# brunohs1993/Nanokappa

Measured on AMD Instinct MI355X. Metric: phonon-steps/sec (whole node), higher is better.
Workload: dtype f64

## Files before the change

nanokappa_amd/csrc/nk_engine.hip:

```cpp
#include <hip/hip_runtime.h>
#include <dlfcn.h>
#include <math.h>
#include <stdio.h>
#include <stdlib.h>
#include <string.h>
#include <algorithm>
#include <functional>
#include <queue>
#include <string>
#include <type_traits>
#include <chrono>
#include <time.h>
#include <vector>

#include <rccl/rccl.h>

#include "../../include/nanokappa_hip.h"
#include "nk_kernels.h"
#include "nk_field.h"
#include "nk_modes.h"
#include "nk_group.h"
#include "nk_freepath.h"
#include "nk_freecols.h"
#ifndef NK_PLAIN_IN_ENGINE
// ... 1957 lines not shown
}

static size_t nk_events_lds(nk_ctx *ctx, size_t lds_g) {
    NkDev &d = ctx->d;
    size_t lds_ev = lds_g;
    if (!(d.qx && nk_geom_mode(ctx) == 2 && d.NG > 0 && d.tree_nfam > 0)) return lds_ev;
    const size_t off = (lds_g + 15) & ~(size_t)15, fixed = off + (size_t)NK_EVENTS_PEND * NK_EV_WG * 4 + 1024;
    size_t budget = (size_t)160 * 1024 / NK_EV_PER_CU > fixed ? (size_t)160 * 1024 / NK_EV_PER_CU - fixed : 0;
    if (const char *e = getenv("NK_EVENTS_TREE_LDS")) { const size_t v = (size_t)atol(e); if (v < budget) budget = v; }
    for (int l = 0; l <= d.tree_top; ++l) {
        const int fam0 = d.tree_base[l] >> 2;
        const size_t bytes = (size_t)(d.tree_nfam - fam0) * NK_TREE_FAMILY_FLOATS * 4;
        if (bytes <= budget) { d.tree_lds_fam0 = fam0; d.tree_lds_off = (int32_t)off; lds_ev = off + bytes; break; }
    }
    if (getenv("NK_VERBOSE") && ctx->timing.batches <= 1)
        fprintf(stderr, "[nanokappa_hip] k_events: families %d .. %d of the face tree in LDS (%zu B of %zu B per workgroup)\n", d.tree_lds_fam0, d.tree_nfam, lds_ev - off, lds_ev);
    return lds_ev;
}
static int nk_side_tallies(nk_ctx *ctx, int s, std::vector<int> &band_s) {
    const int64_t stepno = ctx->step + s;
    if (!nk_flux_step(ctx, stepno)) return NK_OK;
    const int nranks = ctx->comm ? ctx->comm_nranks : 1;
    if (ctx->band_B > 0) {
        NK_TRY(nk_band_pass(ctx, false, ctx->band_rows_d + band_s.size() * 4 * (size_t)ctx->d.S * ctx->band_B));
        band_s.push_back(s);
    }
    if (ctx->field.on && nk_nth_step(ctx->field.cfg.every, stepno)) {
        NK_TRY(nk_field_sample(ctx, false, false));
        NK_HIP(nk_field_accumulate(ctx->field.g, ctx->field, nranks, ctx->stream));
        if (ctx->fgroups.on) {
            NK_TRY(nk_field_sample(ctx, true, false));
            NK_HIP(nk_field_accumulate(ctx->fgroups.g, ctx->field, nranks, ctx->stream));
        }
    }
    if (ctx->modes.on && nk_nth_step(ctx->modes.cfg.every, stepno)) {
        NK_TRY(nk_modes_sample(ctx, false));
        NK_HIP(nk_modes_accumulate(ctx->modes, nranks, ctx->num_cu, ctx->stream));
    }
    return NK_OK;
}
static int nk_band_collect(nk_ctx *ctx, const std::vector<int> &band_s, int32_t nd) {
    if (band_s.empty()) return NK_OK;
    const size_t rl = 4 * (size_t)ctx->d.S * ctx->band_B;
    std::vector<double> br(band_s.size() * rl);
    NK_HIP(hipMemcpyAsync(br.data(), ctx->band_rows_d, br.size() * sizeof(double), hipMemcpyDeviceToHost, ctx->stream));
    NK_HIP(hipStreamSynchronize(ctx->stream));
    const int unseen = ctx->halt_words[2] ? nd - 1 : -1;
    for (size_t r = 0; r < band_s.size(); ++r) {
        if (band_s[r] >= nd || band_s[r] == unseen) continue;
        ctx->band_rows.insert(ctx->band_rows.end(), br.begin() + r * rl, br.begin() + (r + 1) * rl);
        ctx->band_steps.push_back(ctx->step + band_s[r]);
    }
    return NK_OK;
}
static int nk_batch_timing(nk_ctx *ctx, int nev, int32_t nsteps, int32_t nd) {
    const hipEvent_t *ev = ctx->evpool.data();
    float ms = 0.f;
    double sk = 0.0, ek = 0.0, vk = 0.0;
    const int nt = nd < nev ? nd : nev;
    for (int s = 0; s < nt; ++s) {
        NK_HIP(hipEventElapsedTime(&ms, ev[4 * s], ev[4 * s + 1])); ek += ms;
        NK_HIP(hipEventElapsedTime(&ms, ev[4 * s + 1], ev[4 * s + 2])); sk += ms;
        NK_HIP(hipEventElapsedTime(&ms, ev[4 * s + 2], ev[4 * s + 3])); vk += ms;
    }
    NK_HIP(hipEventElapsedTime(&ms, ev[64], ev[65]));
    if (nt > 0 && nd == nsteps) {
        ctx->timing.step_kernel_ms = sk / nt;
        ctx->timing.emit_kernel_ms = ek / nt;
        ctx->timing.events_kernel_ms = vk / nt;
        ctx->timing.total_ms = ms;
    }
    return NK_OK;
}
#ifdef NK_STAMPS
#include "nk_stamps.h"
#endif

static int nk_step_batch(nk_ctx *ctx, int32_t nsteps, std::vector<double> &h, int32_t *done) {
    NkDev &d = ctx->d;
    const int R = d.R, NB = d.NB;
    NkBatch b;
    NK_TRY(nk_batch_enter(ctx, nsteps, b));
    const size_t lds_g = nk_lds(ctx, true), lds_w = nk_lds(ctx, true, d.pid ? 3 : 2), lds_e = nk_lds(ctx, true, 1);
    const size_t lds_t = lds_e > (size_t)(NK_WG * 8 + 16) ? lds_e : (size_t)(NK_WG * 8 + 16);
    const size_t lds_ev = nk_events_lds(ctx, lds_g);
    const int gm_ = nk_geom_mode(ctx);
    const bool rough_ = d.Fr > 0, rbf_ = d.sv_interp == 3, pid_ = (bool)d.pid, split_ = d.qx != nullptr;
    const bool lrec_ = nk_want_lrec(ctx);
    const int g_sweep = b.g_sweep, g_emit = b.g_emit;
    const int g_ev = split_ ? ctx->num_cu * NK_EV_PER_CU : 0;
    const int rows = g_sweep + g_ev;
    const int nev = nsteps < 4 ? 0 : 4;
    NK_TRY(nk_batch_events(ctx));
    hipEvent_t *ev = ctx->evpool.data();
    NK_HIP(hipEventRecord(ev[64], ctx->stream));
    std::vector<int> band_s;
    if (ctx->band_B > 0) {
        int nflux = 0;
        for (int s = 0; s < nsteps; ++s) nflux += nk_flux_step(ctx, ctx->step + s) ? 1 : 0;
        if (nflux > 0) NK_TRY(nk_band_ensure(ctx, nflux));
    }
    for (int s = 0; s < nsteps; ++s) {
        NK_TRY(nk_batch_prelude(ctx, b, s));
        const NkGroupRec rec = nk_batch_rec(ctx, b, s);
        const uint32_t step = rec.step;
        const int do_flux = rec.do_flux;
        if (s < nev) NK_HIP(hipEventRecord(ev[4 * s], ctx->stream));
        if (R > 0 && d.res_gen == 2) k_emit_one_to_one<<<ctx->num_cu * 4, NK_WG, 0, ctx->stream>>>(d, step);
        if (R > 0 && !b.emitted_ahead) NK_EMIT_LAUNCH(k_emit, g_emit, lds_e, d, step);
        if (s < nev) NK_HIP(hipEventRecord(ev[4 * s + 1], ctx->stream));
        if (b.alt) ctx->walked = true;
        d.down = rec.down;
        NK_SWEEP_DISPATCH(gm_, rough_, rbf_, pid_, split_, lrec_, (KERNEL<<<g_sweep, NK_WG, lds_w, ctx->stream>>>(d, step, rec.do_relax, do_flux)));
        d.down = 0;
        if (split_) {
            k_events_begin<<<1, 1024, 0, ctx->stream>>>(d);
            const int64_t ev_key = (int64_t)lds_ev * 64 + (gm_ | (rough_ << 2) | (rbf_ << 3) | (pid_ << 4));
            if (ctx->ev_lds_set != ev_key) {
                hipError_t ea_ = hipSuccess;
                NK_EVENTS_DISPATCH(gm_, rough_, rbf_, pid_, (ea_ = hipFuncSetAttribute((const void *)KERNEL, hipFuncAttributeMaxDynamicSharedMemorySize, (int)lds_ev)));
                NK_HIP(ea_);
                ctx->ev_lds_set = ev_key;
            }
            NK_EVENTS_DISPATCH(gm_, rough_, rbf_, pid_, (KERNEL<<<g_ev, NK_EV_WG, lds_ev, ctx->stream>>>(d, step, do_flux, g_sweep)));
            k_events_end<<<(d.nseg + 255) / 256, 256, 0, ctx->stream>>>(d);
        }
        if (d.mig_buf) k_deliver<<<g_emit, NK_WG, 0, ctx->stream>>>(d, 1);
        if (s < nev) NK_HIP(hipEventRecord(ev[4 * s + 2], ctx->stream));
        NK_TRY(nk_side_tallies(ctx, s, band_s));
        double *hrow = rec.hist_row;
        const bool ahead = b.tail_emit;
        if (ctx->comm) {
            if (ahead) NK_EMIT_LAUNCH(k_tail, NB + g_emit, lds_t, d, step + 1u, rows, ctx->acc, hrow, do_flux, 0, NB);
            else k_reduce<<<NB, NK_WG, 0, ctx->stream>>>(d, rows, ctx->acc, hrow, do_flux, 0);
            ncclResult_t nrc = ctx->rccl.AllReduce(ctx->acc, ctx->acc, (size_t)NB + 2, ncclDouble, ncclSum, ctx->comm, ctx->stream);
            if (nrc != ncclSuccess) { ctx->err = "ncclAllReduce failed"; return NK_ERR_COMM; }
            k_update<<<1, NK_WG, 0, ctx->stream>>>(d, ctx->acc, hrow, do_flux);
        } else if (ahead) {
            NK_EMIT_LAUNCH(k_tail, NB + g_emit, lds_t, d, step + 1u, rows, ctx->acc, hrow, do_flux, 1, NB);
        } else {
            k_reduce<<<NB, NK_WG, 0, ctx->stream>>>(d, rows, ctx->acc, hrow, do_flux, 1);
        }
        b.emitted_ahead = ahead;
        if (s < nev) NK_HIP(hipEventRecord(ev[4 * s + 3], ctx->stream));
        if ((s & 63) == 0) NK_HIP(hipGetLastError());
    }
    NK_HIP(hipEventRecord(ev[65], ctx->stream));
    NK_HIP(hipGetLastError());
    if (nsteps <= 4) { hipError_t q_; while ((q_ = hipStreamQuery(ctx->stream)) == hipErrorNotReady) { } if (q_ != hipSuccess) { ctx->err = std::string("hipStreamQuery: ") + hipGetErrorString(q_); return NK_ERR_HIP; } }
    NK_HIP(hipStreamSynchronize(ctx->stream));
    NK_TRY(nk_batch_collect(ctx, nsteps, h, done));
#ifdef NK_STAMPS
    NK_TRY(nk_stamps_report(ctx));
#endif
    NK_TRY(nk_band_collect(ctx, band_s, *done));
    nk_batch_leave(ctx, b, nsteps, *done);
    return nk_batch_timing(ctx, nev, nsteps, *done);
}

static inline bool nk_want_resident(const nk_ctx *ctx) {
    const NkDev &d = ctx->d;
    if (!getenv("NK_RESIDENT") || getenv("NK_NO_RESIDENT") || ctx->comm || d.nranks != 1 || d.Fr > 0 || d.mig_buf || d.qx || nk_geom_mode(ctx) != 1) return false;
    if (ctx->band_B > 0) return false;
    if (ctx->field.on) return false;
    if (ctx->modes.on) return false;
    if (d.res_gen == 2 || d.sv_interp == 3 || d.NB > 254 || d.S > 128 || d.nseg <= 0) return false;
    const int64_t lim = getenv("NK_RESIDENT_MAX") ? atoll(getenv("NK_RESIDENT_MAX")) : 1200000;
// ... 213 lines not shown
    int R = 0;
    std::vector<nk_ctx *> m;
    int device = 0;
    std::string err;
    unsigned char *dev = nullptr;
    unsigned char *stage = nullptr;
    NkGroupRec *recs_d = nullptr, *recs_h = nullptr;
    int recs_cap = 0;
    std::vector<hipEvent_t> ev;
    std::vector<char> halted, alone;
    nk_group_report rep = {};
};
static thread_local std::string g_group_error;

#define NK_GHIP(call)                                                                                  \
    do {                                                                                               \
        hipError_t e_ = (call);                                                                        \
        if (e_ != hipSuccess) {                                                                        \
            g->err = std::string(#call) + ": " + hipGetErrorString(e_);                                \
            return NK_ERR_HIP;                                                                         \
        }                                                                                              \
    } while (0)

struct NkGroupKey {
    NkGroupKind kind;
    int S, R, NB, flux_every, contains_every, res_gen;
    double dt;
    int64_t step;
};
static NkGroupKey nk_group_key(nk_ctx *ctx) {
    const NkDev &d = ctx->d;
    NkGroupKey k;
    k.kind.pid = (bool)d.pid;
    k.kind.lrec = nk_want_lrec(ctx);
    k.kind.fast = k.kind.pid ? 0 : nk_sweep_fast(ctx);
    k.kind.box = d.box != 0;
    k.S = d.S; k.R = d.R; k.NB = d.NB;
    k.flux_every = ctx->params.flux_every; k.contains_every = ctx->params.contains_every; k.res_gen = d.res_gen;
    k.dt = d.dt;
    k.step = ctx->step;
    return k;
}
struct NkGroupPlan { NkGroupKey key; size_t lds_w = 0, lds_t = 0; int device = 0; };
static std::string nk_group_scope(nk_ctx *ctx) {
    const NkDev &d = ctx->d;
    if (!(ctx->have_material && ctx->have_mesh && ctx->have_sv && ctx->have_params)) return "it is not ready (engine not configured: need material, mesh, subvolumes and params)";
    if (ctx->comm || d.nranks != 1) return "it belongs to a communicator (several ranks)";
    if (d.Fr > 0 || d.mig_buf) return "it has rough facets (their migrants are delivered between the sweep and the tail)";
    if (nk_geom_mode(ctx) != 1) return "its mesh is too large for tables in LDS";
    if (nk_want_split(ctx) || d.qx) return "it uses the split sweep";
    if (d.sv_interp == 3) return "it uses RBF temperatures";
    if (d.res_gen == 2) return "its generator is 'one_to_one'";
    if (ctx->band_B > 0) return "its band-resolved flux is on (nk_set_bands)";
    if (ctx->field.on) return "its field maps are on (nk_set_field)";
    if (ctx->modes.on) return "its mode tally is on (nk_set_modes)";
    if (d.R > 0 && getenv("NK_NO_TAIL_EMIT")) return "NK_NO_TAIL_EMIT is set (the emission would need a launch of its own)";
    return "";
}
static int nk_group_check(nk_ctx *const *m, int R, NkGroupPlan *plan, std::string &err) {
    if (R < 1 || R > NK_GROUP_MAX_MEMBERS) { err = "nk_group: R = " + std::to_string(R) + " is outside 1 .. " + std::to_string(NK_GROUP_MAX_MEMBERS); return NK_ERR_ARG; }
    if (!m) { err = "nk_group: NULL members"; return NK_ERR_ARG; }
    for (int r = 0; r < R; ++r) {
        if (!m[r]) { err = "nk_group: member " + std::to_string(r) + " is NULL"; return NK_ERR_ARG; }
        for (int q = 0; q < r; ++q)
            if (m[q] == m[r]) { err = "nk_group: member " + std::to_string(r) + " is the same context as member " + std::to_string(q) + " (given twice)"; return NK_ERR_ARG; }
    }
    for (int r = 1; r < R; ++r)
        if (m[r]->device != m[0]->device) {
            err = "nk_group: member " + std::to_string(r) + " is on device " + std::to_string(m[r]->device) + ", member 0 on device " + std::to_string(m[0]->device);
            return NK_ERR_ARG;
        }
    for (int r = 0; r < R; ++r) {
        const std::string why = nk_group_scope(m[r]);
        if (!why.empty()) { err = "nk_group: member " + std::to_string(r) + " is outside the grouped path: " + why; return NK_ERR_ARG; }
    }
    for (int r = 0; r < R; ++r) {
        if (nk_check_ready(m[r])) { err = "nk_group: member " + std::to_string(r) + " is not ready: " + m[r]->err; return NK_ERR_ARG; }
        const std::string why = nk_group_scope(m[r]);
        if (!why.empty()) { err = "nk_group: member " + std::to_string(r) + " is outside the grouped path: " + why; return NK_ERR_ARG; }
    }
    size_t lds_w = 0, lds_t = 0;
    for (int r = 0; r < R; ++r) {
        const size_t w = nk_lds(m[r], true, m[r]->d.pid ? 3 : 2), e = nk_lds(m[r], true, 1);
        const size_t tl = e > (size_t)(NK_WG * 8 + 16) ? e : (size_t)(NK_WG * 8 + 16);
        if (w > 64 * 1024 || tl > 64 * 1024) { err = "nk_group: member " + std::to_string(r) + " is outside the grouped path: its tables need more than 64 KB of LDS"; return NK_ERR_ARG; }
        lds_w = std::max(lds_w, w); lds_t = std::max(lds_t, tl);
    }
    const NkGroupKey k0 = nk_group_key(m[0]);
    for (int r = 1; r < R; ++r) {
        const NkGroupKey k = nk_group_key(m[r]);
        const char *what = nullptr;
        std::string a, b;
#define NK_GROUP_SAME(field, name) if (!what && !(k.field == k0.field)) { what = name; a = std::to_string(k.field); b = std::to_string(k0.field); }
        NK_GROUP_SAME(step, "current step")
        NK_GROUP_SAME(S, "subvolumes")
        NK_GROUP_SAME(R, "reservoirs")
        NK_GROUP_SAME(NB, "tally bins")
        NK_GROUP_SAME(flux_every, "flux_every")
        NK_GROUP_SAME(contains_every, "contains_every")
        NK_GROUP_SAME(dt, "dt")
        NK_GROUP_SAME(res_gen, "generator")
        NK_GROUP_SAME(kind.pid, "kernel instantiation (particle ids)")
        NK_GROUP_SAME(kind.lrec, "kernel instantiation (mode records in LDS)")
        NK_GROUP_SAME(kind.fast, "kernel instantiation (subvolume fast path)")
        NK_GROUP_SAME(kind.box, "kernel instantiation (box store)")
#undef NK_GROUP_SAME
        if (what) {
            err = "nk_group: member " + std::to_string(r) + " disagrees with member 0 on the " + what + " (" + a + " against " + b + ")";
            return NK_ERR_ARG;
        }
    }
    if (plan) { plan->key = k0; plan->lds_w = lds_w; plan->lds_t = lds_t; plan->device = m[0]->device; }
    return NK_OK;
}

int nk_group_create(nk_group **out, nk_ctx *const *members, int32_t R) {
    if (!out) { g_group_error = "nk_group_create: NULL out"; return NK_ERR_ARG; }
    *out = nullptr;
    NkGroupPlan plan;
    int rc = nk_group_check(members, R, &plan, g_group_error);
    if (rc) return rc;
    const int device = plan.device;
    nk_group *g = new nk_group();
    g->R = R;
    g->m.assign(members, members + R);
    g->halted.assign((size_t)R, 0);
    g->alone.assign((size_t)R, 0);
    g->device = device;
    g->rep.R = R;
    const size_t bytes = sizeof(NkGroupHead) + (size_t)NK_GROUP_MAX * sizeof(NkDev);
    hipError_t e = hipSetDevice(device);
    if (e == hipSuccess) e = hipMalloc((void **)&g->dev, bytes);
    if (e == hipSuccess) e = hipHostMalloc((void **)&g->stage, bytes, hipHostMallocDefault);
    if (e == hipSuccess) {
        g->ev.resize(3 * 4 + 2);
        for (auto &v : g->ev) { v = nullptr; if (e == hipSuccess) e = hipEventCreate(&v); }
    }
    if (e != hipSuccess) {
        g_group_error = std::string("nk_group_create: ") + hipGetErrorString(e);
        (void)hipGetLastError();
        nk_group_destroy(g);
        return NK_ERR_HIP;
    }
    *out = g;
    return NK_OK;
}

void nk_group_destroy(nk_group *g) {
    if (!g) return;
    (void)hipSetDevice(g->device);
    for (auto &v : g->ev) if (v) hipEventDestroy(v);
    if (g->dev) hipFree(g->dev);
    if (g->stage) hipHostFree(g->stage);
    if (g->recs_d) hipFree(g->recs_d);
    if (g->recs_h) hipHostFree(g->recs_h);
    delete g;
}

const char *nk_group_last_error(const nk_group *g) { return g ? g->err.c_str() : g_group_error.c_str(); }

int nk_group_info(nk_group *g, nk_group_report *out) {
    if (!g || !out) { if (g) g->err = "nk_group_info: NULL argument"; return NK_ERR_ARG; }
    *out = g->rep;
    return NK_OK;
}

static int nk_member_failed(nk_group *g, int r, int rc) {
// ... 1329 lines not shown
```

nanokappa_amd/csrc/nk_group.hip:

```cpp
#include <hip/hip_runtime.h>
#include <stdint.h>
#include "../../include/nanokappa_hip.h"
#define NK_KERNEL_LINKAGE template <int NK_NOT_IN_THIS_TU = 0>
#include "nk_kernels.h"
#include "nk_group.h"

#define NK_CONSTANT_AS __attribute__((address_space(4)))

__device__ __forceinline__ int nk_group_member(const NK_CONSTANT_AS int32_t *pre, int b) {
    int r = 0;
#pragma unroll
    for (int k = 1; k < NK_GROUP_MAX; ++k) r += (b >= pre[k]) ? 1 : 0;
    return r;
}
__device__ __forceinline__ void nk_group_dev(NkDev &d, const NkDev *devs, int r) {
    const NK_CONSTANT_AS NkDev *c = (const NK_CONSTANT_AS NkDev *)devs + r;
    __builtin_memcpy(&d, c, sizeof(NkDev));
}

template <bool PID, bool LREC, int FAST, bool BOX>
__global__ __launch_bounds__(NK_WG, NK_SWEEP_BOUND(1, false, false, false)) void k_sweep_group(const NkGroupHead *head_, const NkDev *devs,
                                                                                               const NkGroupRec *recs_) {
    extern __shared__ __align__(16) unsigned char smem[];
    const NK_CONSTANT_AS NkGroupHead *head = (const NK_CONSTANT_AS NkGroupHead *)head_;
    const int b = (int)blockIdx.x;
    const int r = nk_group_member(head->pre_sweep, b);
    const int wg = b - head->pre_sweep[r], nwg = head->pre_sweep[r + 1] - head->pre_sweep[r];
    const NK_CONSTANT_AS NkGroupRec *rec = (const NK_CONSTANT_AS NkGroupRec *)recs_ + r;
    NkDev d;
    nk_group_dev(d, devs, r);
    if (d.halt[0]) return;
    d.down = rec->down;
    if (FAST) { d.sv_kind = 0; d.sv_interp = FAST - 1; d.T_ref_local = 1; }
    NkLds L;
    nk_lds_setup<1, PID ? 3 : 2>(d, smem, L);
    nk_sweep_body<1, false, false, PID, false, LREC, FAST, BOX>(d, L, rec->step, rec->do_relax, rec->do_flux, wg, nwg);
    nk_lds_flush(d, L, wg);
}

#ifdef NK_GROUP_PLAIN

#define NK_GROUP_SWEEP(P, L, F, B) k_sweep_group<P, L, F, B><<<grid, NK_WG, lds, stream>>>(head, devs, recs)
hipError_t nk_group_launch_sweep_fast(const NkGroupKind &k, int grid, size_t lds, hipStream_t stream, const NkGroupHead *head, const NkDev *devs,
                                      const NkGroupRec *recs) {
    if (k.pid || (k.fast != 1 && k.fast != 2)) return hipErrorInvalidValue;
    if (k.box) {
        if (k.lrec) { if (k.fast == 1) NK_GROUP_SWEEP(false, true, 1, true); else NK_GROUP_SWEEP(false, true, 2, true); }
        else { if (k.fast == 1) NK_GROUP_SWEEP(false, false, 1, true); else NK_GROUP_SWEEP(false, false, 2, true); }
    } else {
        if (k.lrec) { if (k.fast == 1) NK_GROUP_SWEEP(false, true, 1, false); else NK_GROUP_SWEEP(false, true, 2, false); }
        else { if (k.fast == 1) NK_GROUP_SWEEP(false, false, 1, false); else NK_GROUP_SWEEP(false, false, 2, false); }
    }
    return hipGetLastError();
}

#else

template <bool BOX>
__global__ __launch_bounds__(NK_WG) void k_tail_group(const NkGroupHead *head_, const NkDev *devs, const NkGroupRec *recs_) {
    extern __shared__ __align__(16) unsigned char smem[];
    const NK_CONSTANT_AS NkGroupHead *head = (const NK_CONSTANT_AS NkGroupHead *)head_;
    const int b = (int)blockIdx.x;
    const int r = nk_group_member(head->pre_tail, b);
    const int wg = b - head->pre_tail[r], nwg = head->pre_tail[r + 1] - head->pre_tail[r];
    const int n_reduce = head->NB;
    const NK_CONSTANT_AS NkGroupRec *rec = (const NK_CONSTANT_AS NkGroupRec *)recs_ + r;
    NkDev d;
    nk_group_dev(d, devs, r);
    if (wg < n_reduce) {
        double *sh = reinterpret_cast<double *>(smem);
        int &last = *reinterpret_cast<int *>(smem + NK_WG * sizeof(double));
        nk_reduce_body(d, head->rows[r], rec->acc, rec->hist_row, rec->do_flux, 1, wg, n_reduce, sh, last);
    } else {
        nk_emit_body<1, BOX>(d, rec->step + 1u, smem, wg - n_reduce, nwg - n_reduce, true);
    }
}

#define NK_GROUP_SWEEP(P, L, B) k_sweep_group<P, L, 0, B><<<grid, NK_WG, lds, stream>>>(head, devs, recs)
hipError_t nk_group_launch_sweep(const NkGroupKind &k, int grid, size_t lds, hipStream_t stream, const NkGroupHead *head, const NkDev *devs,
                                 const NkGroupRec *recs) {
    if (k.fast) return nk_group_launch_sweep_fast(k, grid, lds, stream, head, devs, recs);
    if (k.box) {
        if (k.pid) { if (k.lrec) NK_GROUP_SWEEP(true, true, true); else NK_GROUP_SWEEP(true, false, true); }
        else { if (k.lrec) NK_GROUP_SWEEP(false, true, true); else NK_GROUP_SWEEP(false, false, true); }
    } else {
        if (k.pid) { if (k.lrec) NK_GROUP_SWEEP(true, true, false); else NK_GROUP_SWEEP(true, false, false); }
        else { if (k.lrec) NK_GROUP_SWEEP(false, true, false); else NK_GROUP_SWEEP(false, false, false); }
    }
    return hipGetLastError();
}

hipError_t nk_group_launch_tail(bool box, int grid, size_t lds, hipStream_t stream, const NkGroupHead *head, const NkDev *devs, const NkGroupRec *recs) {
    if (box) k_tail_group<true><<<grid, NK_WG, lds, stream>>>(head, devs, recs);
    else k_tail_group<false><<<grid, NK_WG, lds, stream>>>(head, devs, recs);
    return hipGetLastError();
}

#endif
```

nanokappa_amd/csrc/nk_kernels.h:

```cpp
#pragma once
#ifndef NK_KERNEL_LINKAGE
#define NK_KERNEL_LINKAGE
#endif
#include "nk_device.h"

#define NK_TILE 64
#ifndef NK_NT
#define NK_NT 0
#endif
#if NK_NT
#define NK_LD(p) __builtin_nontemporal_load(p)
#define NK_ST(p, v) __builtin_nontemporal_store(v, p)
#else
#define NK_LD(p) (*(p))
#define NK_ST(p, v) (*(p) = (v))
#endif
#ifdef NK_STAMPS
#define NK_STAMP(k)                                                                                    \
    do {                                                                                               \
        unsigned long long t_;                                                                         \
        __builtin_amdgcn_sched_barrier(0);                                                             \
        asm volatile("s_memtime %0\n\ts_waitcnt lgkmcnt(0)" : "=s"(t_)::"memory");                     \
        __builtin_amdgcn_sched_barrier(0);                                                             \
        st_acc[k] += t_ - st_last;                                                                     \
// ... 1176 lines not shown
            o[3] = t1 - st_t0; o[4] = st_walk; o[5] = (st_got << 32) | st_pass; o[6] = (st_nleaf << 40) | st_leaf;
        }
    }
#endif
    nk_lds_flush(d, L, row0 + blockIdx.x);
}

NK_KERNEL_LINKAGE __global__ __launch_bounds__(NK_WG) void k_anchor(NkDev d, int honor_halt) {
    if (!d.seg_lo || (honor_halt && d.halt[0])) return;
    const int lane = threadIdx.x & 63, wave = threadIdx.x >> 6;
    const int nwaves = gridDim.x * (NK_WG / 64);
    for (int seg = blockIdx.x * (NK_WG / 64) + wave; seg < d.nseg; seg += nwaves) {
        const int lo = d.seg_lo[seg];
        if (lo <= 0) continue;
        const int64_t base = (int64_t)seg * d.segcap;
        int n = d.seg_count[seg] + (d.R > 0 ? d.seg_new[seg] : 0);
        n = lo + n <= d.segcap ? n : d.segcap - lo;
        for (int j0 = 0; j0 < n; j0 += 64) {
            const bool on = j0 + lane < n;
            const NkSlot qs = nk_slot(d, base + lo + j0 + (on ? lane : 0)), qd = nk_slot(d, base + j0 + (on ? lane : 0));
            double vx = 0, vy = 0, vz = 0, vo = 0, vn = 0;
            uint32_t vw = 0u;
            uint64_t vp = 0;
            if (on) {
                vx = d.x.p[qs.od]; vy = d.y.p[qs.od]; vz = d.z.p[qs.od]; vo = d.occ.p[qs.od]; vw = d.w0.p[qs.ow];
                if (d.nts.p) vn = d.nts.p[qs.od];
                if (d.pid.p) vp = d.pid.p[qs.od];
            }
            asm volatile("s_waitcnt vmcnt(0)" ::: "memory");
            __builtin_amdgcn_fence(__ATOMIC_SEQ_CST, "wavefront");
            if (on) {
                d.x.p[qd.od] = vx; d.y.p[qd.od] = vy; d.z.p[qd.od] = vz; d.occ.p[qd.od] = vo; d.w0.p[qd.ow] = vw;
                if (d.nts.p) d.nts.p[qd.od] = vn;
                if (d.pid.p) d.pid.p[qd.od] = vp;
            }
            asm volatile("s_waitcnt vmcnt(0)" ::: "memory");
        }
        if (lane == 0) d.seg_lo[seg] = 0;
    }
}

NK_KERNEL_LINKAGE __global__ __launch_bounds__(NK_WG) void k_regrow(NkDev o, NkDev n) {
    for (int seg = blockIdx.x; seg < o.nseg; seg += gridDim.x) {
        const int cnt = o.seg_count[seg];
        const int64_t a = (int64_t)seg * o.segcap, b = (int64_t)seg * n.segcap;
        for (int i = threadIdx.x; i < cnt; i += blockDim.x) {
            n.x[b + i] = o.x[a + i]; n.y[b + i] = o.y[a + i]; n.z[b + i] = o.z[a + i];
            n.occ[b + i] = o.occ[a + i]; if (o.nts && n.nts) n.nts[b + i] = o.nts[a + i];
            n.w0[b + i] = o.w0[a + i];
            if (o.pid && n.pid) n.pid[b + i] = o.pid[a + i];
        }
        if (threadIdx.x == 0) n.seg_count[seg] = cnt;
    }
}

NK_KERNEL_LINKAGE __global__ __launch_bounds__(NK_WG) void k_deliver(NkDev d, int in_step) {
    const int lane = threadIdx.x & 63, wave = __builtin_amdgcn_readfirstlane(threadIdx.x >> 6);
    const int nwaves = gridDim.x * (NK_WG / 64);
    for (int seg = blockIdx.x * (NK_WG / 64) + wave; seg < d.nseg; seg += nwaves) {
        int n = d.mig_n[seg];
        if (n <= 0) continue;
        if (n > d.mig_cap) n = d.mig_cap;
        const int count = d.seg_count[seg];
        const int lo = d.seg_lo ? d.seg_lo[seg] : 0;
        if (lo + count + n > d.segcap) { if (lane == 0 && !in_step) { atomicOr(d.halt + 2, 1); atomicOr(d.halt, 1); } continue; }
        const int64_t base = (int64_t)seg * d.segcap + lo + count;
        for (int j = lane; j < n; j += 64) {
            const double2 *r = d.mig_buf + ((int64_t)seg * d.mig_cap + j) * 4;
            const double2 a = r[0], b = r[1], c = r[2], e = r[3];
            d.x[base + j] = a.x; d.y[base + j] = a.y; d.z[base + j] = b.x; d.occ[base + j] = b.y; if (d.nts) d.nts[base + j] = c.x;
            d.pid[base + j] = (uint64_t)__double_as_longlong(c.y);
            d.w0[base + j] = (uint32_t)__double_as_longlong(e.x);
        }
        if (lane == 0) {
            d.seg_count[seg] = count + n;
            d.mig_n[seg] = 0;
            const int bound = d.R > 0 ? d.seg_bound[seg] : 0;
            if ((int64_t)lo + count + n + 2 * (bound + 2 * n) + NK_TILE > (int64_t)d.segcap) atomicOr(d.halt + 1, 1);
            if (2 * n > d.mig_cap) atomicOr(d.halt + 3, 1);
        }
    }
}

__device__ __forceinline__ void nk_update_sv(const NkDev &d, double Eraw, double Ns, double Told, int t, double Ta, double Tb, double Tz,
                                             double Ea, double Ez, double &Tnew_out, double &E_out) {
    const int n = d.nE;
        double norm;
        if (d.norm_fixed) norm = d.active_modes / (d.particle_density * d.sv_volume[t]);
        else { norm = d.active_modes / Ns; if (isnan(norm)) norm = 0.0; }
        double E = Eraw * norm / d.QV;
        int it = (int)((Told - Ta) / (Tb - Ta));
        it = it < 0 ? 0 : (it > n - 1 ? n - 1 : it);
        int base = it - 1;
        base = base < 0 ? 0 : (base > n - 4 ? n - 4 : base);
        double wT[4], wE[4];
#pragma unroll
        for (int j = 0; j < 4; ++j) { const int q = n >= 4 ? base + j : 0; wT[j] = d.Tarr[q]; wE[j] = d.Earr[q]; }
        double ref;
        if (Told < Ta) ref = Ea;
        else if (Told > Tz) ref = Ez;
        else if (n >= 4 && wT[0] < Told && !(wT[3] < Told)) {
            const int c = (wT[1] < Told) + (wT[2] < Told);
            const double xlo = c == 0 ? wT[0] : (c == 1 ? wT[1] : wT[2]), xhi = c == 0 ? wT[1] : (c == 1 ? wT[2] : wT[3]);
            const double ylo = c == 0 ? wE[0] : (c == 1 ? wE[1] : wE[2]), yhi = c == 0 ? wE[1] : (c == 1 ? wE[2] : wE[3]);
            ref = (yhi - ylo) / (xhi - xlo) * (Told - xlo) + ylo;
        } else { int io; ref = nk_interp_lin_hint(d.Tarr, d.Earr, n, Told, it, io); }
        E += ref;
        double Tnew;
        if (E < Ea) Tnew = d.Tfill_lo;
        else if (E > Ez) Tnew = d.Tfill_hi;
        else if (n >= 4 && wE[0] < E && !(wE[3] < E)) {
            const int c = (wE[1] < E) + (wE[2] < E);
            const double xlo = c == 0 ? wE[0] : (c == 1 ? wE[1] : wE[2]), xhi = c == 0 ? wE[1] : (c == 1 ? wE[2] : wE[3]);
            const double ylo = c == 0 ? wT[0] : (c == 1 ? wT[1] : wT[2]), yhi = c == 0 ? wT[1] : (c == 1 ? wT[2] : wT[3]);
            Tnew = (yhi - ylo) / (xhi - xlo) * (E - xlo) + ylo;
        } else { int io; Tnew = nk_interp_lin_hint(d.Earr, d.Tarr, n, E, it, io); }
        Tnew_out = Tnew;
        E_out = E;
}
__device__ __forceinline__ void nk_update_body(const NkDev &d, const double *acc, double *hist_row, int do_flux) {
    const int tid = threadIdx.x, nth = blockDim.x;
    const int S = d.S, NB = d.NB, n = d.nE;
    const double Ta = d.Tarr[0], Tb = d.Tarr[1], Tz = d.Tarr[n - 1], Ea = d.Earr[0], Ez = d.Earr[n - 1];
    for (int t = tid; t < S; t += nth) {
        double Tnew, E;
        nk_update_sv(d, acc[t], acc[S + t], d.T_ref_local ? d.T_sv[t] : d.T_ref, t, Ta, Tb, Tz, Ea, Ez, Tnew, E);
        hist_row[NB + t] = Tnew;
        hist_row[NB + S + t] = E;
        d.T_sv[t] = Tnew;
    }
    for (int b = tid; b < NB; b += nth) hist_row[b] = acc[b];
    if (d.sv_interp == 3) {
        __syncthreads();
        const int P = d.rbf_P;
        for (int j = tid; j < P; j += nth) {
            double a = 0.0;
            for (int i = 0; i < S; ++i) a += d.rbf_inv[(int64_t)j * P + i] * d.T_sv[i];
            d.T_sv[S + j] = a;
        }
    }
    if (d.res_gen == 2) for (int r = tid; r < d.R; r += nth) d.nleave_prev[r] = (int32_t)acc[5 * S + r];
    if (tid == 0) {
        hist_row[NB + 2 * S + 0] = (double)do_flux;
        hist_row[NB + 2 * S + 1] = 1.0;
        const bool hdel = acc[NB + 1] > 0.0;
        const bool hreq = acc[NB] > 0.0 || hdel;
        hist_row[NB + 2 * S + 2] = hreq ? 1.0 : 0.0;
        hist_row[NB + 2 * S + 3] = (double)*d.overflow;
        if (hreq) d.halt[0] = 1;
        if (hdel) d.halt[2] = 1;
        hist_row[NB + 2 * S + 4] = hreq ? 1.0 : 0.0;
        hist_row[NB + 2 * S + 5] = (double)d.halt[1];
        hist_row[NB + 2 * S + 6] = (hdel || d.halt[2]) ? 1.0 : 0.0;
        hist_row[NB + 2 * S + 7] = (double)d.halt[3];
    }
}

__device__ __forceinline__ void nk_reduce_body(const NkDev &d, int rows, double *acc, double *hist_row, int do_flux, int fuse, int b,
                                               int nblocks, double *sh, int &last) {
    if (d.halt[0]) return;
    const int NB = d.NB;
    double v = 0.0;
    for (int r = threadIdx.x; r < rows; r += NK_WG) v += d.partials[(int64_t)r * NB + b];
    sh[threadIdx.x] = v;
    __syncthreads();
    for (int o = NK_WG / 2; o > 0; o >>= 1) {
        if (threadIdx.x < o) sh[threadIdx.x] += sh[threadIdx.x + o];
        __syncthreads();
    }
    if (threadIdx.x == 0) acc[b] = sh[0];
    if (b == 0) {
        int stuck = 0;
        if (d.mig_n) for (int sg = threadIdx.x; sg < d.nseg; sg += NK_WG) { const int n = d.mig_n[sg]; stuck |= (n > 0 && d.seg_count[sg] + (n < d.mig_cap ? n : d.mig_cap) > d.segcap) ? 1 : 0; }
        stuck = __syncthreads_or(stuck);
        if (threadIdx.x == 0) { acc[NB] = (double)d.halt[1]; acc[NB + 1] = (double)stuck; }
    }
    if (!fuse) return;
    if (threadIdx.x == 0) {
        __threadfence();
        last = (atomicAdd(d.ticket, 1) == nblocks - 1);
    }
    __syncthreads();
    if (!last) return;
    if (threadIdx.x == 0) *d.ticket = 0;
    __threadfence();
    nk_update_body(d, acc, hist_row, do_flux);
}
NK_KERNEL_LINKAGE __global__ __launch_bounds__(NK_WG) void k_reduce(NkDev d, int rows, double *acc, double *hist_row, int do_flux, int fuse) {
    __shared__ double sh[NK_WG];
    __shared__ int last;
    nk_reduce_body(d, rows, acc, hist_row, do_flux, fuse, (int)blockIdx.x, (int)gridDim.x, sh, last);
}
template <int GEOM, bool BOX = false>
__global__ __launch_bounds__(NK_WG) void k_tail(NkDev d, uint32_t step_next, int rows, double *acc, double *hist_row, int do_flux, int fuse,
                                                int n_reduce) {
    extern __shared__ __align__(16) unsigned char smem[];
    if ((int)blockIdx.x < n_reduce) {
        double *sh = reinterpret_cast<double *>(smem);
        int &last = *reinterpret_cast<int *>(smem + NK_WG * sizeof(double));
        nk_reduce_body(d, rows, acc, hist_row, do_flux, fuse, (int)blockIdx.x, n_reduce, sh, last);
    } else {
        nk_emit_body<GEOM, BOX>(d, step_next, smem, (int)blockIdx.x - n_reduce, (int)gridDim.x - n_reduce, true);
    }
}

__device__ __forceinline__ bool nk_wait_word(const unsigned int *w, unsigned int atleast) {
    int spins = 0;
    while (__hip_atomic_load(w, __ATOMIC_RELAXED, __HIP_MEMORY_SCOPE_AGENT) < atleast) {
        __builtin_amdgcn_s_sleep(1);
        if (++spins > 1000000) return false;
    }
    return true;
}
template <bool BOX, bool PID, bool LREC>
__global__ __launch_bounds__(NK_WG, 2) void k_resident(NkDev d, uint32_t step0, int nsteps, int relax0, int flux_every, double *hist, int hrow,
                                                       unsigned int *bar) {
    extern __shared__ __align__(16) unsigned char smem[];
    if (d.halt[0]) return;
    NkLds L;
    nk_lds_setup<1, PID ? 5 : 4>(d, smem, L);
    const int tid = threadIdx.x, wg = (int)blockIdx.x, G = (int)gridDim.x;
    const int S = d.S, R = d.R, NB = d.NB, a = d.sv_axis;
    double *Tsv = const_cast<double *>(L.tb.Tsv);
    NkSv *sv = const_cast<NkSv *>(L.tb.sv);
    const int nE = d.nE;
    const double Ta = d.Tarr[0], Tb = d.Tarr[1], Tz = d.Tarr[nE - 1], Ea = d.Earr[0], Ez = d.Earr[nE - 1];
    unsigned int *flags = bar + 32, *flagsT = bar + 32 + 1024;
    unsigned long long *rows = reinterpret_cast<unsigned long long *>(d.partials);
    unsigned long long *Tpub = reinterpret_cast<unsigned long long *>(d.T_sv);
    const int NBP = (NB + 1) & ~1;
    unsigned long long *dbg = reinterpret_cast<unsigned long long *>(bar + 8);
#ifdef NK_STAMPS
    if (R > 0) nk_emit_segments<1, BOX>(d, L, step0, wg, G, false, 0ull, 0ull);
#else
    if (R > 0) nk_emit_segments<1, BOX>(d, L, step0, wg, G, false);
#endif
    for (int s = 0; s < nsteps; ++s) {
        const uint32_t step = step0 + (uint32_t)s;
        const int do_flux = (flux_every > 0 && ((step + 1u) % (uint32_t)flux_every) == 0u) ? 1 : 0;
        const bool mark = s == nsteps - 1 && tid == 0 && (wg == 0 || wg == G / 2);
        unsigned long long *mk = dbg + (wg == 0 ? 0 : 8);
        if (mark) mk[0] = __builtin_amdgcn_s_memrealtime();
#ifdef NK_STAMPS
        nk_sweep_body<1, false, false, PID, false, LREC, 0, BOX>(d, L, step, s == 0 ? relax0 : 1, do_flux, wg, G, 0ull);
#else
        nk_sweep_body<1, false, false, PID, false, LREC, 0, BOX>(d, L, step, s == 0 ? relax0 : 1, do_flux, wg, G);
#endif
        unsigned long long *rows_s = rows + (size_t)(s & 1) * G * NBP;
        __syncthreads();
        if (mark) mk[1] = __builtin_amdgcn_s_memrealtime();
        for (int b = tid; b < NB; b += NK_WG) {
            double v = 0.0;
            if (b < S) { for (int r = 0; r < NK_NREP; ++r) v += L.bins.E[r * S + b]; }
            else if (b < 2 * S) { unsigned int c = 0; for (int r = 0; r < NK_NREP; ++r) c += L.bins.N[r * S + (b - S)]; v = (double)c; }
            else if (b < 5 * S) { const int k = b - 2 * S; for (int r = 0; r < NK_NREP; ++r) v += L.bins.flux[r * 3 * S + k]; }
            else if (b < 5 * S + R) v = (double)L.bins.nleave[b - 5 * S];
            else if (b < 5 * S + 2 * R) v = L.bins.resb[4 * (b - 5 * S - R)];
            else if (b < 5 * S + 5 * R) { const int k = b - 5 * S - 2 * R; v = L.bins.resb[4 * (k / 3) + 1 + (k % 3)]; }
            else v = (double)L.bins.misc[0];
            __hip_atomic_store(rows_s + (size_t)wg * NBP + b, (unsigned long long)__double_as_longlong(v), __ATOMIC_RELAXED, __HIP_MEMORY_SCOPE_AGENT);
        }
        if (tid == 0 && NBP > NB) __hip_atomic_store(rows_s + (size_t)wg * NBP + NB, 0ull, __ATOMIC_RELAXED, __HIP_MEMORY_SCOPE_AGENT);
        asm volatile("s_waitcnt vmcnt(0) lgkmcnt(0)" ::: "memory");
        __builtin_amdgcn_fence(__ATOMIC_RELEASE, "workgroup");
        __syncthreads();
        if (tid == 0) __hip_atomic_store(flags + wg, (unsigned int)(s + 1), __ATOMIC_RELAXED, __HIP_MEMORY_SCOPE_AGENT);
        for (int i = tid; i < NK_NREP * S; i += NK_WG) { L.bins.E[i] = 0.0; L.bins.N[i] = 0u; }
        for (int i = tid; i < NK_NREP * 3 * S; i += NK_WG) L.bins.flux[i] = 0.0;
        for (int i = tid; i < 4 * R; i += NK_WG) L.bins.resb[i] = 0.0;
        for (int i = tid; i < R; i += NK_WG) L.bins.nleave[i] = 0u;
        if (tid == 0) L.bins.misc[0] = 0u;
        __syncthreads();
        if (mark && wg == 0) mk[2] = __builtin_amdgcn_s_memrealtime();
#ifdef NK_STAMPS
        if (R > 0 && s + 1 < nsteps) nk_emit_segments<1, BOX>(d, L, step + 1u, wg, G, true, 0ull, 0ull);
#else
        if (R > 0 && s + 1 < nsteps) nk_emit_segments<1, BOX>(d, L, step + 1u, wg, G, true);
#endif
        int ok = 1, hreq = 0;
        if (mark) mk[wg == 0 ? 3 : 2] = __builtin_amdgcn_s_memrealtime();
        double *hrowp = hist + (size_t)s * hrow;
        const int ntask = S + (NB - 2 * S);
// ... 848 lines not shown
```

Baseline: 53.54 billion.

## Let each reduce block own its column's update instead of last-block ticket

The fused reduce path no longer uses a global ticket so that the last block runs the whole temperature/energy update. Each reduce block now sums its own bin column together with the matching Ns column, then computes that subvolume's new temperature and energy and writes its hist entries directly. Halt is recorded as a per-step token so blocks of the same step keep going. The column sum loads four rows at a time to overlap memory latency, and the reduce LDS scratch doubles to hold the second column. This removes a serial tail and a device-wide fence/atomic, at the cost of more complex halt semantics and relaxed-load ordering assumptions.

```diff
diff --git a/nanokappa_amd/csrc/nk_engine.hip b/nanokappa_amd/csrc/nk_engine.hip
--- a/nanokappa_amd/csrc/nk_engine.hip
+++ b/nanokappa_amd/csrc/nk_engine.hip
@@ -2063,7 +2063,7 @@
     NkBatch b;
     NK_TRY(nk_batch_enter(ctx, nsteps, b));
     const size_t lds_g = nk_lds(ctx, true), lds_w = nk_lds(ctx, true, d.pid ? 3 : 2), lds_e = nk_lds(ctx, true, 1);
-    const size_t lds_t = lds_e > (size_t)(NK_WG * 8 + 16) ? lds_e : (size_t)(NK_WG * 8 + 16);
+    const size_t lds_t = lds_e > (size_t)(2 * NK_WG * 8 + 16) ? lds_e : (size_t)(2 * NK_WG * 8 + 16);
     const size_t lds_ev = nk_events_lds(ctx, lds_g);
     const int gm_ = nk_geom_mode(ctx);
     const bool rough_ = d.Fr > 0, rbf_ = d.sv_interp == 3, pid_ = (bool)d.pid, split_ = d.qx != nullptr;
@@ -2443,7 +2443,7 @@
     size_t lds_w = 0, lds_t = 0;
     for (int r = 0; r < R; ++r) {
         const size_t w = nk_lds(m[r], true, m[r]->d.pid ? 3 : 2), e = nk_lds(m[r], true, 1);
-        const size_t tl = e > (size_t)(NK_WG * 8 + 16) ? e : (size_t)(NK_WG * 8 + 16);
+        const size_t tl = e > (size_t)(2 * NK_WG * 8 + 16) ? e : (size_t)(2 * NK_WG * 8 + 16);
         if (w > 64 * 1024 || tl > 64 * 1024) { err = "nk_group: member " + std::to_string(r) + " is outside the grouped path: its tables need more than 64 KB of LDS"; return NK_ERR_ARG; }
         lds_w = std::max(lds_w, w); lds_t = std::max(lds_t, tl);
     }
diff --git a/nanokappa_amd/csrc/nk_group.hip b/nanokappa_amd/csrc/nk_group.hip
--- a/nanokappa_amd/csrc/nk_group.hip
+++ b/nanokappa_amd/csrc/nk_group.hip
@@ -68,9 +68,7 @@
     NkDev d;
     nk_group_dev(d, devs, r);
     if (wg < n_reduce) {
-        double *sh = reinterpret_cast<double *>(smem);
-        int &last = *reinterpret_cast<int *>(smem + NK_WG * sizeof(double));
-        nk_reduce_body(d, head->rows[r], rec->acc, rec->hist_row, rec->do_flux, 1, wg, n_reduce, sh, last);
+        nk_reduce_owners(d, head->rows[r], rec->acc, rec->hist_row, rec->do_flux, wg, reinterpret_cast<double *>(smem));
     } else {
         nk_emit_body<1, BOX>(d, rec->step + 1u, smem, wg - n_reduce, nwg - n_reduce, true);
     }
diff --git a/nanokappa_amd/csrc/nk_kernels.h b/nanokappa_amd/csrc/nk_kernels.h
--- a/nanokappa_amd/csrc/nk_kernels.h
+++ b/nanokappa_amd/csrc/nk_kernels.h
@@ -1282,20 +1282,35 @@
     }
 }
 
-__device__ __forceinline__ void nk_update_sv(const NkDev &d, double Eraw, double Ns, double Told, int t, double Ta, double Tb, double Tz,
-                                             double Ea, double Ez, double &Tnew_out, double &E_out) {
+__device__ __forceinline__ int nk_ld_word(const int32_t *p) { return __hip_atomic_load(p, __ATOMIC_RELAXED, __HIP_MEMORY_SCOPE_WAVEFRONT); }
+__device__ __forceinline__ double nk_ld_word(const double *p) { return __hip_atomic_load(p, __ATOMIC_RELAXED, __HIP_MEMORY_SCOPE_WAVEFRONT); }
+struct NkTWin { int it; double T0, T1, T2, T3, E0, E1, E2, E3, vol; };
+template <bool VEC = false>
+__device__ __forceinline__ void nk_update_window(const NkDev &d, double Told, int t, double Ta, double Tb, NkTWin &w) {
     const int n = d.nE;
+    w.vol = d.norm_fixed ? (VEC ? nk_ld_word(d.sv_volume + t) : d.sv_volume[t]) : 1.0;
+    int it = (int)((Told - Ta) / (Tb - Ta));
+    it = it < 0 ? 0 : (it > n - 1 ? n - 1 : it);
+    int base = it - 1;
+    base = base < 0 ? 0 : (base > n - 4 ? n - 4 : base);
+    const int q0 = n >= 4 ? base : 0, q1 = n >= 4 ? base + 1 : 0, q2 = n >= 4 ? base + 2 : 0, q3 = n >= 4 ? base + 3 : 0;
+    if (VEC) {
+        w.T0 = nk_ld_word(d.Tarr + q0); w.T1 = nk_ld_word(d.Tarr + q1); w.T2 = nk_ld_word(d.Tarr + q2); w.T3 = nk_ld_word(d.Tarr + q3);
+        w.E0 = nk_ld_word(d.Earr + q0); w.E1 = nk_ld_word(d.Earr + q1); w.E2 = nk_ld_word(d.Earr + q2); w.E3 = nk_ld_word(d.Earr + q3);
+    } else {
+        w.T0 = d.Tarr[q0]; w.T1 = d.Tarr[q1]; w.T2 = d.Tarr[q2]; w.T3 = d.Tarr[q3];
+        w.E0 = d.Earr[q0]; w.E1 = d.Earr[q1]; w.E2 = d.Earr[q2]; w.E3 = d.Earr[q3];
+    }
+    w.it = it;
+}
+__device__ __forceinline__ void nk_update_sv(const NkDev &d, double Eraw, double Ns, double Told, double Ta, double Tz, double Ea,
+                                             double Ez, const NkTWin &w, double &Tnew_out, double &E_out) {
+    const int n = d.nE, it = w.it;
+    const double wT[4] = {w.T0, w.T1, w.T2, w.T3}, wE[4] = {w.E0, w.E1, w.E2, w.E3};
         double norm;
-        if (d.norm_fixed) norm = d.active_modes / (d.particle_density * d.sv_volume[t]);
+        if (d.norm_fixed) norm = d.active_modes / (d.particle_density * w.vol);
         else { norm = d.active_modes / Ns; if (isnan(norm)) norm = 0.0; }
         double E = Eraw * norm / d.QV;
-        int it = (int)((Told - Ta) / (Tb - Ta));
-        it = it < 0 ? 0 : (it > n - 1 ? n - 1 : it);
-        int base = it - 1;
-        base = base < 0 ? 0 : (base > n - 4 ? n - 4 : base);
-        double wT[4], wE[4];
-#pragma unroll
-        for (int j = 0; j < 4; ++j) { const int q = n >= 4 ? base + j : 0; wT[j] = d.Tarr[q]; wE[j] = d.Earr[q]; }
         double ref;
         if (Told < Ta) ref = Ea;
         else if (Told > Tz) ref = Ez;
@@ -1318,6 +1333,12 @@
         Tnew_out = Tnew;
         E_out = E;
 }
+__device__ __forceinline__ void nk_update_sv(const NkDev &d, double Eraw, double Ns, double Told, int t, double Ta, double Tb, double Tz,
+                                             double Ea, double Ez, double &Tnew_out, double &E_out) {
+    NkTWin w;
+    nk_update_window(d, Told, t, Ta, Tb, w);
+    nk_update_sv(d, Eraw, Ns, Told, Ta, Tz, Ea, Ez, w, Tnew_out, E_out);
+}
 __device__ __forceinline__ void nk_update_body(const NkDev &d, const double *acc, double *hist_row, int do_flux) {
     const int tid = threadIdx.x, nth = blockDim.x;
     const int S = d.S, NB = d.NB, n = d.nE;
@@ -1356,25 +1377,97 @@
     }
 }
 
+__device__ __forceinline__ int nk_halt_token(const double *hist_row) { return (int)((((uintptr_t)hist_row >> 3) << 2) | 2u); }
+__device__ __forceinline__ void nk_column_partial(const NkDev &d, int rows, int b, bool two, int b2, double &v, double &v2) {
+    const int NB = d.NB;
+    v = v2 = 0.0;
+    for (int r0 = threadIdx.x; r0 < rows; r0 += 4 * NK_WG) {
+        double x[4], x2[4];
+#pragma unroll
+        for (int k = 0; k < 4; ++k) {
+            const int r = r0 + k * NK_WG;
+            x[k] = r < rows ? d.partials[(int64_t)r * NB + b] : 0.0;
+            x2[k] = (two && r < rows) ? d.partials[(int64_t)r * NB + b2] : 0.0;
+        }
+#pragma unroll
+        for (int k = 0; k < 4; ++k) if (r0 + k * NK_WG < rows) { v += x[k]; if (two) v2 += x2[k]; }
+    }
+}
+__device__ __forceinline__ void nk_column_tree(double *sh, bool two, double v, double v2) {
+    const int tid = threadIdx.x;
+    sh[tid] = v;
+    if (two) sh[NK_WG + tid] = v2;
+    __syncthreads();
+    for (int o = NK_WG / 2; o > 0; o >>= 1) {
+        if (tid < o) { sh[tid] += sh[tid + o]; if (two) sh[NK_WG + tid] += sh[NK_WG + tid + o]; }
+        __syncthreads();
+    }
+}
+__device__ __forceinline__ int nk_reduce_requests(const NkDev &d, double *acc, int h1) {
+    int stuck = 0;
+    if (d.mig_n) for (int sg = threadIdx.x; sg < d.nseg; sg += NK_WG) { const int n = d.mig_n[sg]; stuck |= (n > 0 && d.seg_count[sg] + (n < d.mig_cap ? n : d.mig_cap) > d.segcap) ? 1 : 0; }
+    stuck = __syncthreads_or(stuck);
+    if (threadIdx.x == 0) { acc[d.NB] = (double)h1; acc[d.NB + 1] = (double)stuck; }
+    return stuck;
+}
+__device__ __forceinline__ void nk_reduce_owners(const NkDev &d, int rows, double *acc, double *hist_row, int do_flux, int b, double *sh) {
+    const int NB = d.NB, S = d.S, tid = threadIdx.x, n = d.nE;
+    const int h_ = nk_ld_word(d.halt);
+    int h1_ = 0, h2_ = 0, h3_ = 0, ovf_ = 0;
+    if (b == 0) { h1_ = nk_ld_word(d.halt + 1); h2_ = nk_ld_word(d.halt + 2); h3_ = nk_ld_word(d.halt + 3); ovf_ = nk_ld_word(d.overflow); }
+    const bool sv = b < S;
+    double Ta = 0.0, Tb = 0.0, Tz = 0.0, Ea = 0.0, Ez = 0.0, Told = 0.0;
+    if (sv) {
+        Ta = nk_ld_word(d.Tarr); Tb = nk_ld_word(d.Tarr + 1); Tz = nk_ld_word(d.Tarr + (n - 1));
+        Ea = nk_ld_word(d.Earr); Ez = nk_ld_word(d.Earr + (n - 1));
+        Told = d.T_ref_local ? nk_ld_word(d.T_sv + b) : d.T_ref;
+    }
+    double v, vN;
+    nk_column_partial(d, rows, b, sv, S + b, v, vN);
+    const int h = __builtin_amdgcn_readfirstlane(h_);
+    if (h && h != nk_halt_token(hist_row)) return;
+    NkTWin w = {};
+    if (sv) nk_update_window<true>(d, Told, b, Ta, Tb, w);
+    nk_column_tree(sh, sv, v, vN);
+    if (tid == 0) {
+        const double s0 = sh[0];
+        acc[b] = s0;
+        hist_row[b] = s0;
+        if (sv) {
+            double Tnew, E;
+            nk_update_sv(d, s0, sh[NK_WG], Told, Ta, Tz, Ea, Ez, w, Tnew, E);
+            hist_row[NB + b] = Tnew;
+            hist_row[NB + S + b] = E;
+            d.T_sv[b] = Tnew;
+        }
+        if (d.res_gen == 2 && b >= 5 * S && b < 5 * S + d.R) d.nleave_prev[b - 5 * S] = (int32_t)s0;
+    }
+    if (b != 0) return;
+    const int h1 = __builtin_amdgcn_readfirstlane(h1_);
+    const int stuck = nk_reduce_requests(d, acc, h1);
+    if (tid == 0) {
+        const bool hdel = stuck != 0, hreq = h1 > 0 || hdel;
+        hist_row[NB + 2 * S + 0] = (double)do_flux;
+        hist_row[NB + 2 * S + 1] = 1.0;
+        hist_row[NB + 2 * S + 2] = hreq ? 1.0 : 0.0;
+        hist_row[NB + 2 * S + 3] = (double)ovf_;
+        if (hreq) d.halt[0] = nk_halt_token(hist_row);
+        if (hdel) d.halt[2] = 1;
+        hist_row[NB + 2 * S + 4] = hreq ? 1.0 : 0.0;
+        hist_row[NB + 2 * S + 5] = (double)h1;
+        hist_row[NB + 2 * S + 6] = (hdel || h2_) ? 1.0 : 0.0;
+        hist_row[NB + 2 * S + 7] = (double)h3_;
+    }
+}
 __device__ __forceinline__ void nk_reduce_body(const NkDev &d, int rows, double *acc, double *hist_row, int do_flux, int fuse, int b,
                                                int nblocks, double *sh, int &last) {
+    if (fuse && d.sv_interp != 3) { nk_reduce_owners(d, rows, acc, hist_row, do_flux, b, sh); return; }
     if (d.halt[0]) return;
-    const int NB = d.NB;
-    double v = 0.0;
-    for (int r = threadIdx.x; r < rows; r += NK_WG) v += d.partials[(int64_t)r * NB + b];
-    sh[threadIdx.x] = v;
-    __syncthreads();
-    for (int o = NK_WG / 2; o > 0; o >>= 1) {
-        if (threadIdx.x < o) sh[threadIdx.x] += sh[threadIdx.x + o];
-        __syncthreads();
-    }
+    double v, v2;
+    nk_column_partial(d, rows, b, false, b, v, v2);
+    nk_column_tree(sh, false, v, v2);
     if (threadIdx.x == 0) acc[b] = sh[0];
-    if (b == 0) {
-        int stuck = 0;
-        if (d.mig_n) for (int sg = threadIdx.x; sg < d.nseg; sg += NK_WG) { const int n = d.mig_n[sg]; stuck |= (n > 0 && d.seg_count[sg] + (n < d.mig_cap ? n : d.mig_cap) > d.segcap) ? 1 : 0; }
-        stuck = __syncthreads_or(stuck);
-        if (threadIdx.x == 0) { acc[NB] = (double)d.halt[1]; acc[NB + 1] = (double)stuck; }
-    }
+    if (b == 0) (void)nk_reduce_requests(d, acc, d.halt[1]);
     if (!fuse) return;
     if (threadIdx.x == 0) {
         __threadfence();
@@ -1387,7 +1480,7 @@
     nk_update_body(d, acc, hist_row, do_flux);
 }
 NK_KERNEL_LINKAGE __global__ __launch_bounds__(NK_WG) void k_reduce(NkDev d, int rows, double *acc, double *hist_row, int do_flux, int fuse) {
-    __shared__ double sh[NK_WG];
+    __shared__ double sh[2 * NK_WG];
     __shared__ int last;
     nk_reduce_body(d, rows, acc, hist_row, do_flux, fuse, (int)blockIdx.x, (int)gridDim.x, sh, last);
 }
@@ -1397,7 +1490,7 @@
     extern __shared__ __align__(16) unsigned char smem[];
     if ((int)blockIdx.x < n_reduce) {
         double *sh = reinterpret_cast<double *>(smem);
-        int &last = *reinterpret_cast<int *>(smem + NK_WG * sizeof(double));
+        int &last = *reinterpret_cast<int *>(smem + 2 * NK_WG * sizeof(double));
         nk_reduce_body(d, rows, acc, hist_row, do_flux, fuse, (int)blockIdx.x, n_reduce, sh, last);
     } else {
         nk_emit_body<GEOM, BOX>(d, step_next, smem, (int)blockIdx.x - n_reduce, (int)gridDim.x - n_reduce, true);
```

After: 53.88 billion (median of 6 runs). No clear change (+0.6%).
